# Total-RD/pymgrid

Hardware: AMD Instinct MI355X
Metric: microgrid env-steps/sec (higher is better)
Workload: dtype f64

## Files before the change

### pymgrid_amd/csrc/mgx_core.hpp

```cpp
#pragma once

#include <hip/hip_runtime.h>
#include <stdint.h>

#include "../../include/mgx.h"

namespace mgx {

enum : int { F_GENSET = 1, F_BATTERY = 2, F_GRID = 4, F_GRID_FIRST = 8 };

enum LogCol : int {
    LC_REWARD = 0, LC_FIXED_PROVIDED, LC_FIXED_ABSORBED, LC_CTRL_PROVIDED, LC_CTRL_ABSORBED,
    LC_OVERALL_PROVIDED, LC_OVERALL_ABSORBED,
    LC_LOAD_MET, LC_RENEWABLE_USED, LC_CURTAILMENT, LC_LOSS_LOAD, LC_OVERGENERATION, LC_UNBALANCED_REWARD,
    LC_COMMON_END,
    LC_GENSET_N = 4, LC_BATTERY_N = 5, LC_GRID_N = 4
};

struct KArgs {
    mgx_columns c;
    int32_t N, T, H, final_step;
    int32_t obs_dim, log_dim;
    int32_t n_load, n_pv;
    int32_t n_genset, n_battery, n_grid;
    int32_t obs_f32;
    int32_t act_f32;
    int32_t obs_state_only;
    int32_t done_bits;
    int32_t obs_colpitch;
    int32_t col_load, col_pv, col_gen, col_bat, col_grid;
    int32_t shaper;
    int32_t noise_increase;
    uint64_t noise_seed;
    int32_t *t_dev;
    int32_t g0, g1;
    const int32_t *grid_final;
    int32_t row_mask;
    int32_t *ep_off, *ep_final;
    int32_t ar_mode;
    int32_t ar_fixed_length, ar_lo, ar_hi, ar_max_length;
    uint64_t ar_seed;
    int32_t *ar_start_io, *ar_length_io, *ar_t0_io;
    void *final_obs;
    int32_t pm_pitch;
};

__device__ __forceinline__ uint8_t done_at(const KArgs &a, int64_t i, int32_t t)
{
    const int32_t fin = a.grid_final ? a.grid_final[i] : a.final_step;
    return (uint8_t)(t >= fin - 1);
}

__device__ __forceinline__ int64_t episode_row(const KArgs &a, int32_t t, int32_t off)
{
    const int64_t row = (int64_t)t + off;
    return row < a.T ? (row < 0 ? 0 : row) : (int64_t)a.T - 1;
}
__device__ __forceinline__ int64_t series_row(const KArgs &a, int64_t i, int32_t t)
{
    return a.ep_off ? episode_row(a, t, a.ep_off[i]) : (int64_t)(t & a.row_mask);
}

__device__ __forceinline__ int32_t resolve_t(const KArgs &a, int32_t t)
{
    if (a.t_dev) {
        const int32_t td = a.t_dev[0] + t;
        if (td >= a.T) { a.t_dev[1] = 1; return a.T - 1; }
        return td;
    }
    return t;
}

__device__ __forceinline__ void advance_counter_in_kernel(const KArgs &a, int32_t k)
{
    if (a.t_dev == nullptr) return;
    __syncthreads();
    if (threadIdx.x == 0) {
        const unsigned prev = atomicAdd((unsigned *)&a.t_dev[2], 1u);
        if (prev == gridDim.x - 1) {
            const int32_t t = __hip_atomic_load(&a.t_dev[0], __ATOMIC_RELAXED, __HIP_MEMORY_SCOPE_AGENT);
            __hip_atomic_store(&a.t_dev[2], 0, __ATOMIC_RELAXED, __HIP_MEMORY_SCOPE_AGENT);
            __hip_atomic_store(&a.t_dev[0], t + k, __ATOMIC_RELEASE, __HIP_MEMORY_SCOPE_AGENT);
        }
    }
}

__device__ __forceinline__ int32_t resolve_t_obs(const KArgs &a, int32_t t) { return a.t_dev ? a.t_dev[0] + t : t; }

__device__ __forceinline__ int32_t resolve_k(const KArgs &a, int32_t t0, int32_t K)
{
    if (a.t_dev && t0 + K > a.T) { a.t_dev[1] = 1; return a.T - t0; }
    return K;
}

struct Params {
    double bat_cmin, bat_cmax, bat_C, bat_D, bat_eta, bat_cost;
    double gen_rmin, gen_rmax, gen_cost, gen_co2, gen_cco2;
    uint32_t gen_times;
    double grid_imp, grid_exp, grid_cco2;
    double ll_cost, og_cost;
};

struct State {
    double charge, soc;
    uint32_t status;
};

struct Derived {
    double bat_lo, bat_sp;
    double gen_sp;
    double grid_lo, grid_sp;
};

struct Inputs {
    double a_goal, a_gen, a_bat, a_grid;
    double load, pv;
    double g_pimp, g_pexp, g_co2, g_stat;
};

struct Outputs {
    double reward;
    double fixed_provided, fixed_absorbed, ctrl_provided, ctrl_absorbed, overall_provided, overall_absorbed;
    double load_met, renewable_used, curtailment, loss_load, overgeneration, unbalanced_reward;
    double genset_production, genset_co2, genset_reward;
    double discharge_amount, charge_amount, battery_reward, soc_pre, charge_pre;
    double grid_import, grid_export, grid_co2, grid_reward;
    uint32_t violations;
};

__device__ __forceinline__ double space_spread(double lo, double hi)
{
    double s = hi - lo;
    return s == 0.0 ? 1.0 : s;
}
__device__ __forceinline__ double space_denorm(double lo, double hi, double v) { return lo + space_spread(lo, hi) * v; }
__device__ __forceinline__ double space_norm(double lo, double hi, double v) { return (v - lo) / space_spread(lo, hi); }

__device__ __forceinline__ double py_min(double a, double b)
{
    double r;
    asm("v_min_f64 %0, %1, %2" : "=v"(r) : "v"(a), "v"(b));
    return r;
}
__device__ __forceinline__ double py_max(double a, double b)
{
    double r;
    asm("v_max_f64 %0, %1, %2" : "=v"(r) : "v"(a), "v"(b));
    return r;
}
__device__ __forceinline__ double py_clip(double x, double lo, double hi) { return py_min(py_max(x, lo), hi); }

template <int F>
__device__ __forceinline__ void derive(const Params &p, Derived &d)
{
    if constexpr (F & F_BATTERY) {
        d.bat_lo = -p.bat_D / p.bat_eta;
        d.bat_sp = space_spread(d.bat_lo, p.bat_C * p.bat_eta);
    }
    if constexpr (F & F_GENSET) d.gen_sp = space_spread(0.0, p.gen_rmax);
    if constexpr (F & F_GRID) {
        d.grid_lo = -1 * p.grid_exp;
        d.grid_sp = space_spread(d.grid_lo, p.grid_imp);
    }
}

constexpr int PP = MGX_PROFILE_PITCH;

__host__ __device__ __forceinline__ bool factorised(const mgx_columns &c) { return c.base_load != nullptr; }

struct GridFactors {
    double lr, pr;
    uint32_t lp, pp, cp, pat;
};

template <int F>
__device__ __forceinline__ void load_factors(const mgx_columns &c, int64_t i, GridFactors &f)
{
// ... 117 lines not shown
}

template <int F>
__device__ __forceinline__ void store_state(const mgx_columns &c, int64_t i, const State &s)
{
    if constexpr (F & F_BATTERY) { c.charge[i] = s.charge; c.soc[i] = s.soc; }
    if constexpr (F & F_GENSET) c.gen_status[i] = s.status;
}

template <int F, typename AT>
__device__ __forceinline__ void load_inputs(const mgx_columns &c, const AT *__restrict__ act,
                                            int64_t N, int64_t i, int64_t t, Inputs &in, int32_t pm = 0)
{
    constexpr int A = 2 * ((F & F_GENSET) != 0) + ((F & F_BATTERY) != 0) + ((F & F_GRID) != 0);
    const AT *a = act + i * A;
    int k = 0;
    if constexpr (F & F_GENSET) { in.a_goal = a[k]; in.a_gen = a[k + 1]; k += 2; }
    if constexpr (F & F_BATTERY) { in.a_bat = a[k]; k += 1; }
    if constexpr (F & F_GRID) { in.a_grid = a[k]; k += 1; }
    if (factorised(c)) {
        GridFactors f;
        load_factors<F>(c, i, f);
        fact_series<F>(c, N, i, t, f, in, pm);
        return;
    }
    if (pm) {
        constexpr int C = (F & F_GRID) ? 6 : 2;
        in.load = c.load_ts[ts_index(pm, N, t, i, C)];
        in.pv = c.pv_ts[ts_index(pm, N, t, i, C)];
        in.g_stat = 1.0;
        if constexpr (F & F_GRID) {
            const double *g = c.grid_ts + grid_ts_index(pm, N, t, 0, i);
            in.g_pimp = g[0]; in.g_pexp = g[1]; in.g_co2 = g[2]; in.g_stat = g[3];
        }
        return;
    }
    in.load = c.load_ts[t * N + i];
    in.pv = c.pv_ts[t * N + i];
    in.g_stat = 1.0;
    if constexpr (F & F_GRID) {
        const double *g = c.grid_ts + (t * 4) * N + i;
        in.g_pimp = g[0]; in.g_pexp = g[N]; in.g_co2 = g[2 * N]; in.g_stat = g[3 * N];
    }
}

__device__ __forceinline__ uint32_t genset_update_status(uint32_t st, uint32_t times, double goal_f)
{
    int cur = st & 0xff, gs = (st >> 8) & 0xff, up = (st >> 16) & 0xff, down = st >> 24;
    const int su = times & 0xff, wd = (times >> 16) & 0xff;
    const bool allow = ((times >> 8) & 1u) == 0;
    const int goal = goal_f > 0.5 ? 1 : 0;
    if (!(goal == cur && cur == gs)) {
        const bool instant = (su == 0 && goal == 1) || (wd == 0 && goal == 0);
        if (goal != gs && (allow || instant)) gs = goal;
        bool finished = false;
        if (up == 0 && gs == 1)        { cur = 1; up = 0;   down = wd; finished = true; }
        else if (down == 0 && gs == 0) { cur = 0; down = 0; up = su;   finished = true; }
        if (!finished) {
            if (goal == cur && cur != gs && allow) {
                gs = goal;
                if (cur) { up = 0; down = wd; } else { down = 0; up = su; }
            } else if (cur == gs && gs != goal) {
                if (cur) { up = 0; down = wd; } else { down = 0; up = su; }
                gs = goal;
            }
            if (gs != cur) { if (gs == 0) down -= 1; else up -= 1; }
        }
    }
    return (uint32_t)cur | ((uint32_t)gs << 8) | ((uint32_t)(up & 0xff) << 16) | ((uint32_t)(down & 0xff) << 24);
}

__device__ __forceinline__ int genset_next_status(uint32_t st, int goal)
{
    const int cur = st & 0xff, up = (st >> 16) & 0xff, down = st >> 24;
    if (goal) return (cur || up == 0) ? 1 : 0;
    return (!cur || down == 0) ? 0 : 1;
}

template <int F>
__device__ __forceinline__ bool genset_wave_is_instant(const Params &p, const State &s)
{
    if constexpr (F & F_GENSET)
        return __all((p.gen_times == 0u) && (s.status == 0u || s.status == 0x0101u)) != 0;
    return false;
}

__device__ __forceinline__ double battery_max_production(const Params &p, double charge)
{
    const double b = charge - p.bat_cmin;
    return py_min(p.bat_D, b) * p.bat_eta;
}
__device__ __forceinline__ double battery_max_consumption(const Params &p, double charge)
{
    const double b = p.bat_cmax - charge;
    return py_min(p.bat_C, b) / p.bat_eta;
}

template <int F, bool HAVE_Q = false>
__device__ __forceinline__ void step_core(const Params &p, const Derived &d, State &s, const Inputs &in, bool normalized,
                                          bool want_soc, bool gen_instant, Outputs &o, double bat_q = 0.0)
{
    double prov = 0.0, absb = 0.0, reward = 0.0;
    uint32_t viol = 0u;

    const double L = -1 * in.load;
    o.load_met = L;
    absb += L; reward += 0.0;
    o.fixed_provided = prov; o.fixed_absorbed = absb;

    if constexpr (F & F_GENSET) {
        if (gen_instant) {
            const uint32_t g = in.a_goal > 0.5 ? 1u : 0u;
            s.status = g | (g << 8);
        } else {
            s.status = genset_update_status(s.status, p.gen_times, in.a_goal);
        }
        const double x = normalized ? 0.0 + d.gen_sp * in.a_gen : in.a_gen;
        const double cur = (double)(s.status & 0xff);
        const double mx = cur * p.gen_rmax, mn = cur * p.gen_rmin;
        const double e = py_clip(x, mn, mx);
        viol |= ((x > mx) || (x < mn) ? 1u : 0u) | (!(in.a_goal >= 0.0 && in.a_goal <= 1.0) ? 8u : 0u) | (x < 0.0 ? 16u : 0u);
        const double co2 = p.gen_co2 * e;
        const double cost = p.gen_cost * e + p.gen_cco2 * co2;
        o.genset_production = e; o.genset_co2 = co2; o.genset_reward = -1.0 * cost;
        prov += e; reward += o.genset_reward;
    }

    auto step_battery = [&]() __attribute__((always_inline)) {
        const double x = normalized ? d.bat_lo + d.bat_sp * in.a_bat : in.a_bat;
        o.soc_pre = s.soc; o.charge_pre = s.charge;
        const bool sink = x < 0;
        const double room = p.bat_cmax - s.charge;
        const double num_sink = py_min(p.bat_C, room);
        const double mp = battery_max_production(p, s.charge);
        const double e_src = py_clip(x, 0.0, mp);
        const double num = sink ? num_sink : -1.0 * e_src;
        double q;
        if constexpr (HAVE_Q) q = bat_q; else q = num / p.bat_eta;
        const double ex = -1.0 * x;
        const double e_sink = py_min(ex, q);
        const double e = sink ? e_sink : e_src;
        viol |= (sink ? (ex > q) : (x > mp)) ? 2u : 0u;
        viol |= !((sink ? e_sink : e_src) >= 0) ? 32u : 0u;
        const double internal = sink ? e * p.bat_eta : ((num < 0) ? q : num * p.bat_eta);
        o.charge_amount = sink ? e : 0.0;
        o.discharge_amount = sink ? 0.0 : e;
        absb += o.charge_amount; prov += o.discharge_amount;
        s.charge = py_max(s.charge + internal, p.bat_cmin);
        if (want_soc) s.soc = s.charge / p.bat_cmax;
        o.battery_reward = -1.0 * (fabs(internal) * p.bat_cost);
        reward += o.battery_reward;
    };
    auto step_grid = [&]() __attribute__((always_inline)) {
        const double x = normalized ? d.grid_lo + d.grid_sp * in.a_grid : in.a_grid;
        const bool sink = x < 0;
        const double ex = -1.0 * x, mc = p.grid_exp * in.g_stat;
        const double e_exp = py_min(ex, mc);
        const double mp = p.grid_imp * in.g_stat;
        const double e_imp = py_clip(x, 0.0, mp);
        viol |= (sink ? (ex > mc) : (x > mp)) ? 4u : 0u;
        viol |= !((sink ? e_exp : e_imp) >= 0) ? 32u : 0u;
        const double co2 = sink ? 0.0 : e_imp * in.g_co2;
        const double cco2 = -1.0 * p.grid_cco2 * co2;
        o.grid_export = sink ? e_exp : 0.0;
        o.grid_import = sink ? 0.0 : e_imp;
        o.grid_co2 = co2;
// ... 1203 lines not shown
```

### pymgrid_amd/csrc/mgx_kernels.hpp

```cpp
#pragma once
#include "mgx_core.hpp"

#include <type_traits>

namespace mgx {

#ifndef MGX_BLOCK
#define MGX_BLOCK 128
#endif
constexpr int BLOCK = MGX_BLOCK;
#ifndef MGX_RING
#define MGX_RING 8
#endif
#ifndef MGX_RING_RICH
#define MGX_RING_RICH 16
#endif
#ifndef MGX_BLOCK_K
#define MGX_BLOCK_K 256
#endif
constexpr int BLOCK_K = MGX_BLOCK_K;
#ifndef MGX_RING_ROLLOUT
#define MGX_RING_ROLLOUT 8
#endif

// ... 168 lines not shown
__global__ __launch_bounds__(BLOCK) void step_kernel(const KArgs a, const void *__restrict__ actions, int32_t t,
                                                     int normalized, double *__restrict__ reward,
                                                     uint8_t *__restrict__ done, void *__restrict__ obs,
                                                     double *__restrict__ log)
{
    t = resolve_t(a, t);
    extern __shared__ __attribute__((aligned(16))) double row_tiles[];
    const int64_t i = (int64_t)a.g0 + (int64_t)blockIdx.x * BLOCK + threadIdx.x;
    if (i < a.g1) step_body<F, EP>(a, actions, t, normalized, reward, done, obs, log, i, row_tiles + (threadIdx.x >> 6) * (64 * ROW_TILE_MAX_D));
    advance_counter_in_kernel(a, 1);
}

template <int F>
__global__ __launch_bounds__(BLOCK) void check_kernel(const KArgs a, const void *__restrict__ actions, int32_t t, int normalized,
                                                      uint32_t *__restrict__ violations)
{
    t = resolve_t(a, t);
    const int64_t i = (int64_t)a.g0 + (int64_t)blockIdx.x * BLOCK + threadIdx.x;
    if (i >= a.g1) return;
    Params p; State s; Inputs in; Outputs o; Derived d;
    load_state<F>(a.c, i, true, s);
    load_params<F>(a.c, i, p);
    derive<F>(p, d);
    const int64_t row = series_row(a, i, t);
    if (a.act_f32) load_inputs<F>(a.c, (const float *)actions, a.N, i, row, in, a.pm_pitch);
    else load_inputs<F>(a.c, (const double *)actions, a.N, i, row, in, a.pm_pitch);
    step_core<F>(p, d, s, in, normalized != 0, false, false, o);
    violations[i] = o.violations;
}

struct FusedOut {
    double *reward;
    uint8_t *done;
    double *soc_trace;
    uint32_t *status_trace;
    double *ret_acc;
    double *log;
};

template <typename AT>
struct RawInputs {
    AT a_goal, a_gen, a_bat, a_grid;
    double load, pv, g_pimp, g_pexp, g_co2, g_stat;
};

template <int F, typename AT>
__device__ __forceinline__ Inputs widen(const RawInputs<AT> &r)
{
    Inputs in;
    if constexpr (F & F_GENSET) { in.a_goal = (double)r.a_goal; in.a_gen = (double)r.a_gen; }
    if constexpr (F & F_BATTERY) in.a_bat = (double)r.a_bat;
    if constexpr (F & F_GRID) {
        in.a_grid = (double)r.a_grid;
        in.g_pimp = r.g_pimp; in.g_pexp = r.g_pexp; in.g_co2 = r.g_co2; in.g_stat = r.g_stat;
    }
    in.load = r.load; in.pv = r.pv;
    return in;
}

template <int F, typename AT>
__device__ __forceinline__ void load_inputs_at(const AT *__restrict__ act, const double *__restrict__ lts,
                                               const double *__restrict__ pts, const double *__restrict__ gts,
                                               int64_t N, int64_t i, int64_t off, RawInputs<AT> &in)
{
    constexpr int A = 2 * ((F & F_GENSET) != 0) + ((F & F_BATTERY) != 0) + ((F & F_GRID) != 0);
    const AT *a = act + off * A;
    int k = 0;
    if constexpr (F & F_GENSET) { in.a_goal = a[k]; in.a_gen = a[k + 1]; k += 2; }
    if constexpr (F & F_BATTERY) { in.a_bat = a[k]; k += 1; }
    if constexpr (F & F_GRID) { in.a_grid = a[k]; k += 1; }
    in.load = lts[off];
    in.pv = pts[off];
    if constexpr (F & F_GRID) {
        const double *g = gts + (4 * off - 3 * i);
        in.g_pimp = g[0]; in.g_pexp = g[N]; in.g_co2 = g[2 * N]; in.g_stat = g[3 * N];
    }
}

#ifndef MGX_FACT_ROWS
#define MGX_FACT_ROWS 128
#endif
constexpr int FACT_ROWS = MGX_FACT_ROWS;

template <int F>
__device__ __forceinline__ void stage_base_rows(const mgx_columns &c, int64_t row0, int32_t n, double *lds, int nthreads)
{
    const int32_t cnt = n * PP;
    const double *__restrict__ bl = c.base_load + row0 * PP;
    const double *__restrict__ bp = c.base_pv + row0 * PP;
    for (int32_t j = threadIdx.x; j < cnt; j += nthreads) {
        lds[j] = bl[j];
        lds[FACT_ROWS * PP + j] = bp[j];
        if constexpr (F & F_GRID) lds[2 * FACT_ROWS * PP + j] = c.base_co2[row0 * PP + j];
    }
}

struct BaseVals { double load, pv, co2; };

template <int F>
__device__ __forceinline__ BaseVals read_base_row(const double *lds, int32_t r, const GridFactors &f)
{
    BaseVals b;
    b.load = lds[r * PP + f.lp];
    b.pv = lds[FACT_ROWS * PP + r * PP + f.pp];
    b.co2 = 0.0;
    if constexpr (F & F_GRID) b.co2 = lds[2 * FACT_ROWS * PP + r * PP + f.cp];
    return b;
}

struct OutageWords {
    uint64_t cur, nxt;
    int64_t wi;
};

__device__ __forceinline__ void outage_init(const mgx_columns &c, int64_t N, int64_t i, int32_t T, int32_t t0, OutageWords &w)
{
    w.wi = t0 >> 6; w.cur = 0; w.nxt = 0;
    if (c.outage_bits) {
        w.cur = c.outage_bits[w.wi * N + i];
        if ((w.wi + 1) * 64 < T) w.nxt = c.outage_bits[(w.wi + 1) * N + i];
    }
}

__device__ __forceinline__ double outage_status(const mgx_columns &c, int64_t N, int64_t i, int32_t T, int32_t row, bool first,
                                                OutageWords &w)
{
    if (!first && (row & 63) == 0) {
        w.cur = w.nxt; w.wi += 1; w.nxt = 0;
        if (c.outage_bits && (w.wi + 1) * 64 < T) w.nxt = c.outage_bits[(w.wi + 1) * N + i];
    }
    return ((w.cur >> (row & 63)) & 1ull) ? 0.0 : 1.0;
}

template <typename AT>
struct RawActions {
    AT a_goal, a_gen, a_bat, a_grid;
};

template <int F, typename AT>
__device__ __forceinline__ void load_actions_at(const AT *__restrict__ row, uint32_t i32, RawActions<AT> &r)
{
    constexpr int A = 2 * ((F & F_GENSET) != 0) + ((F & F_BATTERY) != 0) + ((F & F_GRID) != 0);
    const AT *a = row + i32 * (uint32_t)A;
    int k = 0;
#if MGX_ACT_NT
    if constexpr (F & F_GENSET) { r.a_goal = __builtin_nontemporal_load(a + k); r.a_gen = __builtin_nontemporal_load(a + k + 1); k += 2; }
    if constexpr (F & F_BATTERY) { r.a_bat = __builtin_nontemporal_load(a + k); k += 1; }
    if constexpr (F & F_GRID) { r.a_grid = __builtin_nontemporal_load(a + k); k += 1; }
#else
    if constexpr (F & F_GENSET) { r.a_goal = a[k]; r.a_gen = a[k + 1]; k += 2; }
    if constexpr (F & F_BATTERY) { r.a_bat = a[k]; k += 1; }
    if constexpr (F & F_GRID) { r.a_grid = a[k]; k += 1; }
#endif
}

__device__ __forceinline__ void store_done(const KArgs &a, uint8_t *__restrict__ done, int64_t off, int64_t i, int32_t k, bool dn)
{
    if (a.done_bits) {
        const unsigned long long b = __ballot(dn);
        const int lane = threadIdx.x & 63;
        if ((lane & 15) == 0) {
            const int64_t W = ((int64_t)a.N + 15) >> 4;
            reinterpret_cast<uint16_t *>(done)[(int64_t)k * W + (i >> 4)] = (uint16_t)(b >> (lane & 48));
        }
    } else {
        done[off] = (uint8_t)dn;
    }
}

template <int F, int U, typename AT, bool RICH, bool FACT>
__global__ __launch_bounds__(BLOCK_K) void step_k_kernel(const KArgs a, const AT *__restrict__ actions, int32_t t0,
                                                         int32_t K, int normalized, const FusedOut out_rt, int32_t gpb)
{
    FusedOut out = out_rt;
    if constexpr (!RICH) { out.log = nullptr; out.status_trace = nullptr; }
    const int32_t K_launch = K;
    t0 = resolve_t(a, t0);
    K = resolve_k(a, t0, K);
    const int64_t i = (int64_t)a.g0 + (int64_t)blockIdx.x * gpb + threadIdx.x;
    const bool active = (int32_t)threadIdx.x < gpb && i < a.g1;
    if constexpr (!FACT) { if (!active) return; }
    const int64_t N = a.N;
    constexpr int A_DIM = 2 * ((F & F_GENSET) != 0) + ((F & F_BATTERY) != 0) + ((F & F_GRID) != 0);
    Params p; State s; Derived d;
    const bool norm = normalized != 0;
    const bool want_soc = (out.soc_trace != nullptr) || (out.log != nullptr);
    bool gen_instant = false;
    int32_t k_done = 0;
    if (active) {
        load_state<F>(a.c, i, out.log != nullptr, s);
        load_params<F>(a.c, i, p);
        derive<F>(p, d);
        gen_instant = genset_wave_is_instant<F>(p, s);
        k_done = (a.grid_final ? a.grid_final[i] : a.final_step) - 1 - t0;
    }
    double ret = 0.0;

    const bool hot = !RICH && out.reward != nullptr && out.done == nullptr && (!(F & F_BATTERY) || out.soc_trace != nullptr) &&
                     a.shaper == MGX_SHAPER_NONE;
    const uint32_t i32 = (uint32_t)i;
    auto consume = [&](auto gi_tag, auto hot_tag, const Inputs &in, int32_t k, int64_t off) __attribute__((always_inline)) {
        constexpr bool GI = decltype(gi_tag)::value, HOT = decltype(hot_tag)::value;
        Outputs o;
        step_core<F>(p, d, s, in, norm, HOT ? (F & F_BATTERY) != 0 : want_soc, GI, o);
        if constexpr (HOT) {
            const double r = o.reward;
#if MGX_HOT_NT
            __builtin_nontemporal_store(r, (out.reward + (int64_t)k * N) + i32);
            if constexpr (F & F_BATTERY) __builtin_nontemporal_store(s.soc, (out.soc_trace + (int64_t)k * N) + i32);
#else
            (out.reward + (int64_t)k * N)[i32] = r;
            if constexpr (F & F_BATTERY) (out.soc_trace + (int64_t)k * N)[i32] = s.soc;
#endif
            ret += r;
            return;
        }
        const double r = shaped_reward<F>(a.shaper, o);
        {
#if MGX_OUT_NT
            if (out.reward) __builtin_nontemporal_store(r, out.reward + off);
            if (out.done) store_done(a, out.done, off, i, k, k >= k_done);
            if constexpr (F & F_BATTERY) { if (out.soc_trace) __builtin_nontemporal_store(s.soc, out.soc_trace + off); }
            if constexpr (F & F_GENSET) { if (out.status_trace) __builtin_nontemporal_store(s.status, out.status_trace + off); }
#else
            if (out.reward) out.reward[off] = r;
            if (out.done) store_done(a, out.done, off, i, k, k >= k_done);
            if constexpr (F & F_BATTERY) { if (out.soc_trace) out.soc_trace[off] = s.soc; }
            if constexpr (F & F_GENSET) { if (out.status_trace) out.status_trace[off] = s.status; }
#endif
            if (out.log) store_log<F>(out.log + (off - i) * a.log_dim + i, N, o, s.status);
        }
        ret += r;
    };
    auto specialised = [&](auto fn) __attribute__((always_inline)) {
        if constexpr ((F & F_GENSET) != 0) {
            if (gen_instant) { if (hot) fn(std::true_type{}, std::true_type{}); else fn(std::true_type{}, std::false_type{}); }
            else { if (hot) fn(std::false_type{}, std::true_type{}); else fn(std::false_type{}, std::false_type{}); }
        } else {
            if (hot) fn(std::false_type{}, std::true_type{}); else fn(std::false_type{}, std::false_type{});
        }
    };

    if constexpr (FACT) {
        __shared__ double base_lds[((F & F_GRID) ? 3 : 2) * FACT_ROWS * PP];
        static_assert(FACT_ROWS % U == 0, "ring slots are addressed by k % U across LDS chunks");
        GridFactors f;
        f.lr = 0.0; f.pr = 0.0; f.lp = 0u; f.pp = 0u; f.cp = 0u; f.pat = 0u;
        OutageWords ow;
        ow.cur = 0; ow.nxt = 0; ow.wi = 0;
        RawActions<AT> ring[U];
        if (active) {
            load_factors<F>(a.c, i, f);
            if constexpr (F & F_GRID) outage_init(a.c, N, i, a.T, t0, ow);
#pragma unroll
            for (int u = 0; u < U; u++)
                if (u < K) load_actions_at<F>(actions + (int64_t)u * N * A_DIM, i32, ring[u]);
        }
        int64_t off = i;
        auto run_chunk = [&](auto gi_tag, auto hot_tag, int32_t kb, int32_t n) __attribute__((always_inline)) {
            BaseVals nb = read_base_row<F>(base_lds, 0, f);
            for (int32_t k0 = kb; k0 < kb + n; k0 += U) {
#pragma unroll
                for (int u = 0; u < U; u++) {
                    const int32_t k = k0 + u;
                    if (k < kb + n) {
                        const RawActions<AT> ra = ring[u];
                        if (k + U < K) load_actions_at<F>(actions + (int64_t)(k + U) * N * A_DIM, i32, ring[u]);
                        Inputs in;
                        if constexpr (F & F_GENSET) { in.a_goal = (double)ra.a_goal; in.a_gen = (double)ra.a_gen; }
                        if constexpr (F & F_BATTERY) in.a_bat = (double)ra.a_bat;
                        in.load = fact_load(nb.load, f.lr);
                        in.pv = fact_pv(nb.pv, f.pr);
                        if constexpr (F & F_GRID) {
                            in.a_grid = (double)ra.a_grid;
                            in.g_pimp = tariff_price((int32_t)f.pat, t0 + k); in.g_pexp = 0.0;
                            in.g_co2 = nb.co2;
                            in.g_stat = outage_status(a.c, N, i, a.T, t0 + k, k == 0, ow);
                        }
                        const int32_t rn = (k + 1 - kb < n) ? k + 1 - kb : n - 1;
                        nb = read_base_row<F>(base_lds, rn, f);
                        consume(gi_tag, hot_tag, in, k, off);
                        off += N;
                    }
                }
            }
        };
        for (int32_t kb = 0; kb < K; kb += FACT_ROWS) {
            const int32_t n = K - kb < FACT_ROWS ? K - kb : FACT_ROWS;
            __syncthreads();
            stage_base_rows<F>(a.c, (int64_t)t0 + kb, n, base_lds, BLOCK_K);
            __syncthreads();
            if (active) specialised([&](auto gi_tag, auto hot_tag) __attribute__((always_inline)) { run_chunk(gi_tag, hot_tag, kb, n); });
        }
        if (!active) return;
    } else {
        const double *__restrict__ lts = a.c.load_ts + (int64_t)t0 * N;
        const double *__restrict__ pts = a.c.pv_ts + (int64_t)t0 * N;
        const double *__restrict__ gts = (F & F_GRID) ? a.c.grid_ts + (int64_t)t0 * 4 * N : nullptr;
        specialised([&](auto gi_tag, auto hot_tag) __attribute__((always_inline)) {
            RawInputs<AT> ring[U];
#pragma unroll
            for (int u = 0; u < U; u++)
                if (u < K) load_inputs_at<F>(actions, lts, pts, gts, N, i, (int64_t)u * N + i, ring[u]);

            int64_t off = i;
            for (int32_t k0 = 0; k0 < K; k0 += U) {
#pragma unroll
                for (int u = 0; u < U; u++) {
                    const int32_t k = k0 + u;
                    if (k < K) {
                        const Inputs in = widen<F>(ring[u]);
                        if (k + U < K) load_inputs_at<F>(actions, lts, pts, gts, N, i, off + (int64_t)U * N, ring[u]);
                        consume(gi_tag, hot_tag, in, k, off);
                        off += N;
                    }
                }
            }
        });
    }
    if constexpr (F & F_BATTERY) { if (!want_soc) s.soc = s.charge / p.bat_cmax; }
    store_state<F>(a.c, i, s);
    if (out.ret_acc) out.ret_acc[i] += ret;
    advance_counter_in_kernel(a, K_launch);
}

struct FusedLaunch {
    int flags;
    bool act_f32, rich, fact, per_step;
    unsigned blocks;
    hipStream_t stream;
    const KArgs *k;
    const void *actions;
    const PLWords *tab;
    const uint8_t *ids;
    int32_t t, K;
    int normalized;
    FusedOut out;
    int32_t gpb;
};
constexpr int MGX_FUSED_PARTS = 6;
struct MultiStaticLaunch {
    int flags, ng, nb, nr, nl, np;
    unsigned blocks;
    hipStream_t stream;
    const KArgs *k;
    const void *actions;
    int32_t t, K;
    int normalized;
    FusedOut out;
};
bool launch_step_k_multi_static(const MultiStaticLaunch &L);
struct MultiStaticRollout {
    int flags, ng, nb, nr, nl, np;
    unsigned blocks;
    hipStream_t stream;
    const KArgs *k;
    const int32_t *lists;
    int32_t n_lists, list_len;
    const int32_t *ids;
    int per_step;
    int32_t t, K;
    FusedOut out;
};
bool launch_rollout_multi_static(const MultiStaticRollout &L);
bool launch_step_k_p0(const FusedLaunch &L); bool launch_step_k_p1(const FusedLaunch &L); bool launch_step_k_p2(const FusedLaunch &L);
bool launch_step_k_p3(const FusedLaunch &L); bool launch_step_k_p4(const FusedLaunch &L);
bool launch_rollout_p0(const FusedLaunch &L); bool launch_rollout_p1(const FusedLaunch &L); bool launch_rollout_p2(const FusedLaunch &L);
bool launch_rollout_p3(const FusedLaunch &L); bool launch_rollout_p4(const FusedLaunch &L);
enum : int { EP_SRC_FACT = 0, EP_SRC_GRID_MAJOR = 1, EP_SRC_GATHER = 2 };
struct EpisodeLaunch {
    int flags;
    int src;
    bool per_step;
    unsigned blocks;
    int32_t gpb;
    hipStream_t stream;
    const KArgs *k;
    const KArgs *k_dev;
    const PLWords *tab;
    const uint8_t *ids;
    int32_t t, K;
    FusedOut out;
    mgx_episode_stats stats;
};
constexpr int MGX_EPISODE_PARTS = 2;
bool launch_rollout_episodes_p0(const EpisodeLaunch &L); bool launch_rollout_episodes_p1(const EpisodeLaunch &L);
struct StepEpisodeLaunch {
    int flags;
    int src;
    bool act_f32;
    unsigned blocks;
    int32_t gpb;
    hipStream_t stream;
    const KArgs *k;
    const KArgs *k_dev;
    const void *actions;
    int32_t t, K;
    int normalized;
    FusedOut out;
    mgx_episode_stats stats;
};
constexpr int MGX_STEP_EPISODE_PARTS = 2;
bool launch_step_k_episodes_p0(const StepEpisodeLaunch &L); bool launch_step_k_episodes_p1(const StepEpisodeLaunch &L);

template <int F>
// ... 707 lines not shown
#define MGX_FLEET_CASE(FV) case FV: step_discrete_body<FV>(a, tab, (const int32_t *)actions, t, nullptr, reward, done, obs, log, i); break;
        switch (flags) {
            MGX_FLEET_CASE(0) MGX_FLEET_CASE(1) MGX_FLEET_CASE(2) MGX_FLEET_CASE(3) MGX_FLEET_CASE(4)
            MGX_FLEET_CASE(5) MGX_FLEET_CASE(6) MGX_FLEET_CASE(7) MGX_FLEET_CASE(14)
            default: step_discrete_body<15>(a, tab, (const int32_t *)actions, t, nullptr, reward, done, obs, log, i); break;
        }
#undef MGX_FLEET_CASE
        return;
    }
#define MGX_FLEET_CASE(FV) case FV: step_body<FV>(a, actions, t, fa.normalized, reward, done, obs, log, i); break;
    switch (flags) {
        MGX_FLEET_CASE(0) MGX_FLEET_CASE(1) MGX_FLEET_CASE(2) MGX_FLEET_CASE(3) MGX_FLEET_CASE(4)
        MGX_FLEET_CASE(5) MGX_FLEET_CASE(6) MGX_FLEET_CASE(7) MGX_FLEET_CASE(14)
        default: step_body<15>(a, actions, t, fa.normalized, reward, done, obs, log, i); break;
    }
#undef MGX_FLEET_CASE
}

struct FleetHead {
    const PLWords *tab;
    int64_t n_grids;
    int32_t t, flags, pad0, pad1;
};
struct FleetBucket {
    FleetHead hd;
    KArgs k;
    const void *actions;
    double *reward; uint8_t *done; void *obs; double *log;
};
struct FleetArgsV {
    int32_t n, normalized, pad0, pad1;
    FleetBucket b[MGX_FLEET_MAX];
};
static_assert(sizeof(FleetArgsV) <= 3840, "the kernarg segment holds 4 KB");

#define MGX_FLEET_V_HEAD \
    typedef const char __attribute__((address_space(4))) *kernarg_bytes; \
    const kernarg_bytes mine = (kernarg_bytes)__builtin_amdgcn_kernarg_segment_ptr() + offsetof(FleetArgsV, b) \
                               + (size_t)blockIdx.y * sizeof(FleetBucket); \
    typedef uint32_t u32x8 __attribute__((ext_vector_type(8))); \
    static_assert(sizeof(FleetHead) == 32 && offsetof(FleetBucket, hd) == 0, "the head is one s_load_dwordx8"); \
    const u32x8 h8 = *reinterpret_cast<const u32x8 __attribute__((address_space(4))) *>(mine); \
    FleetHead hd; \
    hd.tab = reinterpret_cast<const PLWords *>((uint64_t)h8[0] | ((uint64_t)h8[1] << 32)); \
    hd.n_grids = (int64_t)((uint64_t)h8[2] | ((uint64_t)h8[3] << 32)); \
    hd.t = (int32_t)h8[4]; hd.flags = (int32_t)h8[5]; \
    const int64_t i = (int64_t)blockIdx.x * BLOCK + threadIdx.x; \
    if (i >= hd.n_grids) return; \
    const int normalized = fa.normalized; \
    const FleetBucket &B = *reinterpret_cast<const FleetBucket *>((const char *)mine);

#define MGX_FLEET_V_DISCRETE(FV, EPV) case FV: { step_discrete_body<FV, EPV>(B.k, *hd.tab, (const int32_t *)B.actions, hd.t, nullptr, B.reward, B.done, B.obs, B.log, i); } break;
#define MGX_FLEET_V_STEP(FV, EPV) case FV: { step_body<FV, EPV>(B.k, B.actions, hd.t, normalized, B.reward, B.done, B.obs, B.log, i); } break;
#define MGX_FLEET_V_SWITCHES(EPV)                                                                                                     \
    if (hd.tab != nullptr) {                                  \
        switch (hd.flags) {                                                                                                           \
            MGX_FLEET_V_DISCRETE(0, EPV) MGX_FLEET_V_DISCRETE(1, EPV) MGX_FLEET_V_DISCRETE(2, EPV) MGX_FLEET_V_DISCRETE(3, EPV)       \
            MGX_FLEET_V_DISCRETE(4, EPV) MGX_FLEET_V_DISCRETE(5, EPV) MGX_FLEET_V_DISCRETE(6, EPV) MGX_FLEET_V_DISCRETE(7, EPV)       \
            MGX_FLEET_V_DISCRETE(14, EPV)                                                                                             \
            default: { step_discrete_body<15, EPV>(B.k, *hd.tab, (const int32_t *)B.actions, hd.t, nullptr, B.reward, B.done, B.obs, B.log, i); } break; \
        }                                                                                                                             \
        return;                                                                                                                       \
    }                                                                                                                                 \
    switch (hd.flags) {                                                                                                               \
        MGX_FLEET_V_STEP(0, EPV) MGX_FLEET_V_STEP(1, EPV) MGX_FLEET_V_STEP(2, EPV) MGX_FLEET_V_STEP(3, EPV) MGX_FLEET_V_STEP(4, EPV)   \
        MGX_FLEET_V_STEP(5, EPV) MGX_FLEET_V_STEP(6, EPV) MGX_FLEET_V_STEP(7, EPV) MGX_FLEET_V_STEP(14, EPV)                          \
        default: { step_body<15, EPV>(B.k, B.actions, hd.t, normalized, B.reward, B.done, B.obs, B.log, i); } break;                  \
    }

template <bool EP>
static __global__ __launch_bounds__(BLOCK) void fleet_step_kernel_v(const FleetArgsV fa)
{
    MGX_FLEET_V_HEAD
    MGX_FLEET_V_SWITCHES(EP)
}

template <int F, int U, bool PER_STEP, bool RICH, bool FACT>
__global__ __launch_bounds__(BLOCK_K) void rollout_kernel(const KArgs a, const PLWords tab, const uint8_t *__restrict__ ids,
                                                          int32_t t0, int32_t K, const FusedOut out_rt, int32_t gpb)
{
    FusedOut out = out_rt;
    if constexpr (!RICH) { out.log = nullptr; out.status_trace = nullptr; }
    const int32_t K_launch = K;
    t0 = resolve_t(a, t0);
    K = resolve_k(a, t0, K);
    const int64_t i = (int64_t)a.g0 + (int64_t)blockIdx.x * gpb + threadIdx.x;
    const bool active = (int32_t)threadIdx.x < gpb && i < a.g1;
    if constexpr (!FACT) { if (!active) return; }
    const int64_t N = a.N;
    Params p; State s; Derived d;
    const bool want_soc = (out.soc_trace != nullptr) || (out.log != nullptr);
    bool gen_instant = false;
    int32_t k_done = 0;
    uint32_t word = 0u;
    if (active) {
        load_state<F>(a.c, i, out.log != nullptr, s);
        load_params<F>(a.c, i, p);
        derive<F>(p, d);
        gen_instant = genset_wave_is_instant<F>(p, s);
        k_done = (a.grid_final ? a.grid_final[i] : a.final_step) - 1 - t0;
        word = PER_STEP ? 0u : pl_select(tab, ids[i]);
    }
    double ret = 0.0;

    const bool hot = !RICH && out.reward != nullptr && out.done == nullptr && (!(F & F_BATTERY) || out.soc_trace != nullptr) &&
                     a.shaper == MGX_SHAPER_NONE;
    const uint32_t i32 = (uint32_t)i;
    auto consume = [&](auto gi_tag, auto hot_tag, Inputs &in, int32_t k, int64_t off) __attribute__((always_inline)) {
        constexpr bool GI = decltype(gi_tag)::value, HOT = decltype(hot_tag)::value;
        double bat_q;
        uint32_t xv = 0u;
        populate_core<F, RICH>(p, s, word, in, bat_q, 0.0 + -1 * in.load, in.pv, GI, &xv);
        Outputs o;
        step_core<F, true>(p, d, s, in, false, HOT ? (F & F_BATTERY) != 0 : want_soc, GI, o, bat_q);
        if constexpr (RICH) o.violations |= xv;
        if constexpr (HOT) {
            const double r = o.reward;
            (out.reward + (int64_t)k * N)[i32] = r;
            if constexpr (F & F_BATTERY) (out.soc_trace + (int64_t)k * N)[i32] = s.soc;
            ret += r;
            return;
        }
        const double r = shaped_reward<F>(a.shaper, o);
        if (out.reward) out.reward[off] = r;
        if (out.done) store_done(a, out.done, off, i, k, k >= k_done);
        if constexpr (F & F_BATTERY) { if (out.soc_trace) out.soc_trace[off] = s.soc; }
        if constexpr (F & F_GENSET) { if (out.status_trace) out.status_trace[off] = s.status; }
        if (out.log) store_log<F>(out.log + (off - i) * a.log_dim + i, N, o, s.status);
        ret += r;
    };
    auto specialised = [&](auto fn) __attribute__((always_inline)) {
        if constexpr ((F & F_GENSET) != 0) {
            if (gen_instant) { if (hot) fn(std::true_type{}, std::true_type{}); else fn(std::true_type{}, std::false_type{}); }
            else { if (hot) fn(std::false_type{}, std::true_type{}); else fn(std::false_type{}, std::false_type{}); }
        } else {
            if (hot) fn(std::false_type{}, std::true_type{}); else fn(std::false_type{}, std::false_type{});
        }
    };
    if constexpr (FACT) {
        __shared__ double base_lds[((F & F_GRID) ? 3 : 2) * FACT_ROWS * PP];
        static_assert(FACT_ROWS % U == 0, "ring slots are addressed by k % U across LDS chunks");
        GridFactors f;
        f.lr = 0.0; f.pr = 0.0; f.lp = 0u; f.pp = 0u; f.cp = 0u; f.pat = 0u;
        OutageWords ow;
        ow.cur = 0; ow.nxt = 0; ow.wi = 0;
        static_assert(U <= 8, "the id ring is one 64-bit register");
        uint64_t idq = 0;
        if (active) {
            load_factors<F>(a.c, i, f);
            if constexpr (F & F_GRID) outage_init(a.c, N, i, a.T, t0, ow);
            if constexpr (PER_STEP) {
#pragma unroll
                for (int u = 0; u < U; u++)
                    if (u < K) idq |= (uint64_t)(ids + (int64_t)u * N)[i32] << (8 * u);
            }
        }
        int64_t off = i;
        auto run_chunk = [&](auto gi_tag, auto hot_tag, int32_t kb, int32_t n) __attribute__((always_inline)) {
            BaseVals nb = read_base_row<F>(base_lds, 0, f);
            for (int32_t k0 = kb; k0 < kb + n; k0 += U) {
#pragma unroll
                for (int u = 0; u < U; u++) {
                    const int32_t k = k0 + u;
                    if (k < kb + n) {
                        if constexpr (PER_STEP) {
                            word = pl_select(tab, (int32_t)((idq >> (8 * u)) & 0xffu));
                            if (k + U < K)
                                idq = (idq & ~(0xffull << (8 * u))) | ((uint64_t)(ids + (int64_t)(k + U) * N)[i32] << (8 * u));
                        }
                        Inputs in;
                        in.load = fact_load(nb.load, f.lr);
                        in.pv = fact_pv(nb.pv, f.pr);
                        in.g_stat = 1.0;
                        if constexpr (F & F_GRID) {
                            in.g_pimp = tariff_price((int32_t)f.pat, t0 + k); in.g_pexp = 0.0;
                            in.g_co2 = nb.co2;
                            in.g_stat = outage_status(a.c, N, i, a.T, t0 + k, k == 0, ow);
                        }
                        const int32_t rn = (k + 1 - kb < n) ? k + 1 - kb : n - 1;
                        nb = read_base_row<F>(base_lds, rn, f);
                        consume(gi_tag, hot_tag, in, k, off);
                        off += N;
                    }
                }
            }
        };
        for (int32_t kb = 0; kb < K; kb += FACT_ROWS) {
            const int32_t n = K - kb < FACT_ROWS ? K - kb : FACT_ROWS;
            __syncthreads();
            stage_base_rows<F>(a.c, (int64_t)t0 + kb, n, base_lds, BLOCK_K);
            __syncthreads();
            if (active) specialised([&](auto gi_tag, auto hot_tag) __attribute__((always_inline)) { run_chunk(gi_tag, hot_tag, kb, n); });
        }
        if (!active) return;
    } else {
        specialised([&](auto gi_tag, auto hot_tag) __attribute__((always_inline)) {
            const double *__restrict__ lts = a.c.load_ts + (int64_t)t0 * N;
            const double *__restrict__ pts = a.c.pv_ts + (int64_t)t0 * N;
            const double *__restrict__ gts = (F & F_GRID) ? a.c.grid_ts + (int64_t)t0 * 4 * N : nullptr;
            Inputs ring[U];
            uint8_t idr[U];
#pragma unroll
            for (int u = 0; u < U; u++)
                if (u < K) {
                    load_series_at<F>(lts, pts, gts, N, i, (int64_t)u * N + i, ring[u]);
                    if constexpr (PER_STEP) idr[u] = ids[(int64_t)u * N + i];
                }

            int64_t off = i;
            for (int32_t k0 = 0; k0 < K; k0 += U) {
#pragma unroll
                for (int u = 0; u < U; u++) {
                    const int32_t k = k0 + u;
                    if (k < K) {
                        Inputs in = ring[u];
                        if constexpr (PER_STEP) word = pl_select(tab, idr[u]);
                        if (k + U < K) {
                            load_series_at<F>(lts, pts, gts, N, i, off + (int64_t)U * N, ring[u]);
                            if constexpr (PER_STEP) idr[u] = ids[off + (int64_t)U * N];
                        }
                        consume(gi_tag, hot_tag, in, k, off);
                        off += N;
                    }
                }
            }
        });
    }
    if constexpr (F & F_BATTERY) { if (!want_soc) s.soc = s.charge / p.bat_cmax; }
    store_state<F>(a.c, i, s);
    if (out.ret_acc) out.ret_acc[i] += ret;
    advance_counter_in_kernel(a, K_launch);
}

constexpr int BLOCK_MULTI = 64;

__device__ __forceinline__ StepLists multi_lists(const KArgs &a, double *lds)
{
    const int cap = multi_list_capacity(a.n_load, a.n_pv, a.n_genset, a.n_battery, a.n_grid);
    StepLists L;
    L.stride = BLOCK_MULTI; L.n_prov = 0; L.n_absb = 0;
    L.prov = lds + threadIdx.x;
    L.absb = lds + (size_t)cap * BLOCK_MULTI + threadIdx.x;
    return L;
}

template <typename OT>
__device__ __forceinline__ void observe_series_multi(const double *__restrict__ ts, int64_t row_stride, int32_t T, int32_t t, int32_t H,
                                                     double lo, double hi, OT *__restrict__ obs, int obs_stride = 1, bool noisy = false,
                                                     double noise_std = 0.0, uint64_t noise_seed = 0, int noise_increase = 0,
                                                     int64_t grid = 0, uint32_t comp = 0)
{
    const double fill = (hi + lo) / 2, sp = space_spread(lo, hi);
    for (int h = 0; h <= H; h++) {
        const bool in = t < T && t + h < T;
        double v = in ? ts[(int64_t)(t + h) * row_stride] : 0.0;
        if (noisy && in && h > 0) {
            const double sd = noise_increase ? noise_std * (1.0 + log(1.0 + (double)(h - 1))) : noise_std;
            v += sd * forecast_normal(noise_seed, grid, comp, t, h);
        }
        obs[h * obs_stride] = (OT)obs_series_value(v, in, h > 0, lo, hi, fill, sp);
    }
}

template <int F, typename OT>
__device__ inline void observe_state_multi(const KArgs &a, int64_t i, OT *__restrict__ dst, int64_t stride)
{
    const int64_t N = a.N;
    int64_t k = 0;
    if constexpr (F & F_GENSET) {
        for (int j = 0; j < a.n_genset; j++) {
            const int64_t c = (int64_t)j * N + i;
            const uint32_t times = a.c.gen_times[c], st = a.c.gen_status[c];
            const double su = (double)(times & 0xff), wd = (double)((times >> 16) & 0xff);
            dst[(k++) * stride] = (OT)space_norm(0.0, 1.0, (double)(st & 0xff));
            dst[(k++) * stride] = (OT)space_norm(0.0, 1.0, (double)((st >> 8) & 0xff));
            dst[(k++) * stride] = (OT)space_norm(0.0, su, (double)((st >> 16) & 0xff));
            dst[(k++) * stride] = (OT)space_norm(0.0, wd, (double)(st >> 24));
        }
    }
    if constexpr (F & F_BATTERY) {
        for (int j = 0; j < a.n_battery; j++) {
            const int64_t c = (int64_t)j * N + i;
            const double cmin = a.c.bat_min_capacity[c], cmax = a.c.bat_max_capacity[c];
            dst[(k++) * stride] = (OT)space_norm(cmin / cmax, 1.0, a.c.soc[c]);
            dst[(k++) * stride] = (OT)space_norm(cmin, cmax, a.c.charge[c]);
        }
    }
}

template <int F, typename OT, bool NOISE = false>
__device__ inline void observe_row_multi(const KArgs &a, int64_t i, int32_t t, OT *__restrict__ obs_row)
{
    const int64_t N = a.N;
    const int W = 1 + a.H;
    int k = (a.n_load + a.n_pv) * W;
    observe_state_multi<F, OT>(a, i, obs_row + k, 1);
    if (a.obs_state_only) return;
    k = 0;
    const uint64_t nseed = a.noise_seed;
    const int ninc = a.noise_increase;
    for (int j = 0; j < a.n_load; j++, k += W) {
        const bool noisy = NOISE && a.c.load_noise_std != nullptr;
        const double sd = noisy ? a.c.load_noise_std[(int64_t)j * N + i] : 0.0;
        observe_series_multi(a.c.load_ts + (int64_t)j * N + i, (int64_t)a.n_load * N, a.T, t, a.H, a.c.load_lo[(int64_t)j * N + i],
                             a.c.load_hi[(int64_t)j * N + i], obs_row + k, 1, noisy, sd, nseed, ninc, i, (uint32_t)j);
    }
    for (int j = 0; j < a.n_pv; j++, k += W) {
        const bool noisy = NOISE && a.c.pv_noise_std != nullptr;
        const double sd = noisy ? a.c.pv_noise_std[(int64_t)j * N + i] : 0.0;
        observe_series_multi(a.c.pv_ts + (int64_t)j * N + i, (int64_t)a.n_pv * N, a.T, t, a.H, a.c.pv_lo[(int64_t)j * N + i],
                             a.c.pv_hi[(int64_t)j * N + i], obs_row + k, 1, noisy, sd, nseed, ninc, i, (uint32_t)(MGX_MAX_MODULES + j));
    }
    k += 4 * a.n_genset + 2 * a.n_battery;
// ... 1010 lines not shown
```

Baseline: 134.7 billion.

## Hoist prologue loads and base-row staging ahead of state init

Issues the first LDS chunk's global loads into registers at kernel entry. State, params, factors, outage words, action/id rings and ret_acc are then all loaded unconditionally, with inactive lanes clamped to the last valid index, so every load goes out before the first use. This is meant to overlap prologue memory latency and drop the leading barrier. The range and overrun resolution becomes branchless and the overrun flag is written at the end. In exchange it uses more registers for the staged rows, and inactive lanes do redundant loads.

```diff
diff --git a/pymgrid_amd/csrc/mgx_core.hpp b/pymgrid_amd/csrc/mgx_core.hpp
--- a/pymgrid_amd/csrc/mgx_core.hpp
+++ b/pymgrid_amd/csrc/mgx_core.hpp
@@ -93,6 +93,29 @@
     return K;
 }
 
+struct LaunchRange {
+    int32_t t0, K;
+    bool overrun;
+};
+__device__ __forceinline__ LaunchRange resolve_range(const KArgs &a, int32_t t, int32_t K)
+{
+    const bool dc = a.t_dev != nullptr;
+    int32_t tv = 0;
+    if (dc) tv = a.t_dev[0];
+    const int32_t td = tv + t;
+    const bool over_t = dc && td >= a.T;
+    LaunchRange r;
+    r.t0 = over_t ? a.T - 1 : td;
+    const bool over_k = dc && r.t0 + K > a.T;
+    r.K = over_k ? a.T - r.t0 : K;
+    r.overrun = over_t || over_k;
+    return r;
+}
+__device__ __forceinline__ void flag_overrun(const KArgs &a, const LaunchRange &r)
+{
+    if (r.overrun) a.t_dev[1] = 1;
+}
+
 struct Params {
     double bat_cmin, bat_cmax, bat_C, bat_D, bat_eta, bat_cost;
     double gen_rmin, gen_rmax, gen_cost, gen_co2, gen_cco2;
@@ -376,6 +399,13 @@
 {
     if constexpr (F & F_GENSET)
         return __all((p.gen_times == 0u) && (s.status == 0u || s.status == 0x0101u)) != 0;
+    return false;
+}
+template <int F>
+__device__ __forceinline__ bool genset_wave_is_instant(const Params &p, const State &s, bool active)
+{
+    if constexpr (F & F_GENSET)
+        return __all(!active || ((p.gen_times == 0u) && (s.status == 0u || s.status == 0x0101u))) != 0;
     return false;
 }
 
diff --git a/pymgrid_amd/csrc/mgx_kernels.hpp b/pymgrid_amd/csrc/mgx_kernels.hpp
--- a/pymgrid_amd/csrc/mgx_kernels.hpp
+++ b/pymgrid_amd/csrc/mgx_kernels.hpp
@@ -274,16 +274,40 @@
 #endif
 constexpr int FACT_ROWS = MGX_FACT_ROWS;
 
+constexpr int STAGE_PER_THREAD = FACT_ROWS * PP / BLOCK_K;
+static_assert(FACT_ROWS * PP % BLOCK_K == 0, "every thread stages the same number of elements of a chunk");
+
 template <int F>
-__device__ __forceinline__ void stage_base_rows(const mgx_columns &c, int64_t row0, int32_t n, double *lds, int nthreads)
-{
-    const int32_t cnt = n * PP;
+struct StagedRows {
+    double load[STAGE_PER_THREAD], pv[STAGE_PER_THREAD], co2[(F & F_GRID) ? STAGE_PER_THREAD : 1];
+};
+
+template <int F>
+__device__ __forceinline__ void stage_load(const mgx_columns &c, int64_t row0, int32_t n, StagedRows<F> &r)
+{
+    const int32_t last = n * PP - 1;
     const double *__restrict__ bl = c.base_load + row0 * PP;
     const double *__restrict__ bp = c.base_pv + row0 * PP;
-    for (int32_t j = threadIdx.x; j < cnt; j += nthreads) {
-        lds[j] = bl[j];
-        lds[FACT_ROWS * PP + j] = bp[j];
-        if constexpr (F & F_GRID) lds[2 * FACT_ROWS * PP + j] = c.base_co2[row0 * PP + j];
+    const double *__restrict__ bc = (F & F_GRID) ? c.base_co2 + row0 * PP : nullptr;
+#pragma unroll
+    for (int m = 0; m < STAGE_PER_THREAD; m++) {
+        const int32_t j = (int32_t)threadIdx.x + m * BLOCK_K;
+        const int32_t jj = j < last ? j : last;
+        r.load[m] = bl[jj];
+        r.pv[m] = bp[jj];
+        if constexpr (F & F_GRID) r.co2[m] = bc[jj];
+    }
+}
+
+template <int F>
+__device__ __forceinline__ void stage_store(const StagedRows<F> &r, double *lds)
+{
+#pragma unroll
+    for (int m = 0; m < STAGE_PER_THREAD; m++) {
+        const int32_t j = (int32_t)threadIdx.x + m * BLOCK_K;
+        lds[j] = r.load[m];
+        lds[FACT_ROWS * PP + j] = r.pv[m];
+        if constexpr (F & F_GRID) lds[2 * FACT_ROWS * PP + j] = r.co2[m];
     }
 }
 
@@ -367,25 +391,45 @@
     FusedOut out = out_rt;
     if constexpr (!RICH) { out.log = nullptr; out.status_trace = nullptr; }
     const int32_t K_launch = K;
-    t0 = resolve_t(a, t0);
-    K = resolve_k(a, t0, K);
+    const LaunchRange lr = resolve_range(a, t0, K);
+    t0 = lr.t0; K = lr.K;
     const int64_t i = (int64_t)a.g0 + (int64_t)blockIdx.x * gpb + threadIdx.x;
     const bool active = (int32_t)threadIdx.x < gpb && i < a.g1;
     if constexpr (!FACT) { if (!active) return; }
+    const int64_t il = (FACT && i >= a.g1) ? (int64_t)a.g1 - 1 : i;
+    const uint32_t il32 = (uint32_t)il;
     const int64_t N = a.N;
     constexpr int A_DIM = 2 * ((F & F_GENSET) != 0) + ((F & F_BATTERY) != 0) + ((F & F_GRID) != 0);
     Params p; State s; Derived d;
     const bool norm = normalized != 0;
     const bool want_soc = (out.soc_trace != nullptr) || (out.log != nullptr);
-    bool gen_instant = false;
-    int32_t k_done = 0;
-    if (active) {
-        load_state<F>(a.c, i, out.log != nullptr, s);
-        load_params<F>(a.c, i, p);
-        derive<F>(p, d);
-        gen_instant = genset_wave_is_instant<F>(p, s);
-        k_done = (a.grid_final ? a.grid_final[i] : a.final_step) - 1 - t0;
-    }
+    StagedRows<F> staged;
+    if constexpr (FACT) stage_load<F>(a.c, t0, K < FACT_ROWS ? K : FACT_ROWS, staged);
+    load_state<F>(a.c, il, false, s);
+    if constexpr (RICH && (F & F_BATTERY)) {
+        const double soc0 = a.c.soc[il];
+        s.soc = out.log ? soc0 : 0.0;
+    }
+    load_params<F>(a.c, il, p);
+    int32_t fin = a.final_step;
+    if (a.grid_final) fin = a.grid_final[il];
+    double ret0 = 0.0;
+    if constexpr (FACT) { if (out.ret_acc) ret0 = out.ret_acc[il]; }
+    GridFactors f;
+    f.lr = 0.0; f.pr = 0.0; f.lp = 0u; f.pp = 0u; f.cp = 0u; f.pat = 0u;
+    OutageWords ow;
+    ow.cur = 0; ow.nxt = 0; ow.wi = 0;
+    RawActions<AT> ring[FACT ? U : 1];
+    if constexpr (FACT) {
+        load_factors<F>(a.c, il, f);
+        if constexpr (F & F_GRID) outage_init(a.c, N, il, a.T, t0, ow);
+#pragma unroll
+        for (int u = 0; u < U; u++)
+            if (u < K) load_actions_at<F>(actions + (int64_t)u * N * A_DIM, il32, ring[u]);
+    }
+    derive<F>(p, d);
+    const bool gen_instant = genset_wave_is_instant<F>(p, s, active);
+    const int32_t k_done = fin - 1 - t0;
     double ret = 0.0;
 
     const bool hot = !RICH && out.reward != nullptr && out.done == nullptr && (!(F & F_BATTERY) || out.soc_trace != nullptr) &&
@@ -436,18 +480,8 @@
     if constexpr (FACT) {
         __shared__ double base_lds[((F & F_GRID) ? 3 : 2) * FACT_ROWS * PP];
         static_assert(FACT_ROWS % U == 0, "ring slots are addressed by k % U across LDS chunks");
-        GridFactors f;
-        f.lr = 0.0; f.pr = 0.0; f.lp = 0u; f.pp = 0u; f.cp = 0u; f.pat = 0u;
-        OutageWords ow;
-        ow.cur = 0; ow.nxt = 0; ow.wi = 0;
-        RawActions<AT> ring[U];
-        if (active) {
-            load_factors<F>(a.c, i, f);
-            if constexpr (F & F_GRID) outage_init(a.c, N, i, a.T, t0, ow);
-#pragma unroll
-            for (int u = 0; u < U; u++)
-                if (u < K) load_actions_at<F>(actions + (int64_t)u * N * A_DIM, i32, ring[u]);
-        }
+        stage_store<F>(staged, base_lds);
+        __syncthreads();
         int64_t off = i;
         auto run_chunk = [&](auto gi_tag, auto hot_tag, int32_t kb, int32_t n) __attribute__((always_inline)) {
             BaseVals nb = read_base_row<F>(base_lds, 0, f);
@@ -479,9 +513,12 @@
         };
         for (int32_t kb = 0; kb < K; kb += FACT_ROWS) {
             const int32_t n = K - kb < FACT_ROWS ? K - kb : FACT_ROWS;
-            __syncthreads();
-            stage_base_rows<F>(a.c, (int64_t)t0 + kb, n, base_lds, BLOCK_K);
-            __syncthreads();
+            if (kb > 0) {
+                stage_load<F>(a.c, (int64_t)t0 + kb, n, staged);
+                __syncthreads();
+                stage_store<F>(staged, base_lds);
+                __syncthreads();
+            }
             if (active) specialised([&](auto gi_tag, auto hot_tag) __attribute__((always_inline)) { run_chunk(gi_tag, hot_tag, kb, n); });
         }
         if (!active) return;
@@ -512,7 +549,11 @@
     }
     if constexpr (F & F_BATTERY) { if (!want_soc) s.soc = s.charge / p.bat_cmax; }
     store_state<F>(a.c, i, s);
-    if (out.ret_acc) out.ret_acc[i] += ret;
+    if (out.ret_acc) {
+        if constexpr (!FACT) ret0 = out.ret_acc[i];
+        out.ret_acc[i] = ret0 + ret;
+    }
+    flag_overrun(a, lr);
     advance_counter_in_kernel(a, K_launch);
 }
 
@@ -1386,25 +1427,49 @@
     FusedOut out = out_rt;
     if constexpr (!RICH) { out.log = nullptr; out.status_trace = nullptr; }
     const int32_t K_launch = K;
-    t0 = resolve_t(a, t0);
-    K = resolve_k(a, t0, K);
+    const LaunchRange lr = resolve_range(a, t0, K);
+    t0 = lr.t0; K = lr.K;
     const int64_t i = (int64_t)a.g0 + (int64_t)blockIdx.x * gpb + threadIdx.x;
     const bool active = (int32_t)threadIdx.x < gpb && i < a.g1;
     if constexpr (!FACT) { if (!active) return; }
+    const int64_t il = (FACT && i >= a.g1) ? (int64_t)a.g1 - 1 : i;
+    const uint32_t il32 = (uint32_t)il;
     const int64_t N = a.N;
     Params p; State s; Derived d;
     const bool want_soc = (out.soc_trace != nullptr) || (out.log != nullptr);
-    bool gen_instant = false;
-    int32_t k_done = 0;
-    uint32_t word = 0u;
-    if (active) {
-        load_state<F>(a.c, i, out.log != nullptr, s);
-        load_params<F>(a.c, i, p);
-        derive<F>(p, d);
-        gen_instant = genset_wave_is_instant<F>(p, s);
-        k_done = (a.grid_final ? a.grid_final[i] : a.final_step) - 1 - t0;
-        word = PER_STEP ? 0u : pl_select(tab, ids[i]);
-    }
+    StagedRows<F> staged;
+    if constexpr (FACT) stage_load<F>(a.c, t0, K < FACT_ROWS ? K : FACT_ROWS, staged);
+    load_state<F>(a.c, il, false, s);
+    if constexpr (RICH && (F & F_BATTERY)) {
+        const double soc0 = a.c.soc[il];
+        s.soc = out.log ? soc0 : 0.0;
+    }
+    load_params<F>(a.c, il, p);
+    int32_t fin = a.final_step;
+    if (a.grid_final) fin = a.grid_final[il];
+    double ret0 = 0.0;
+    if constexpr (FACT) { if (out.ret_acc) ret0 = out.ret_acc[il]; }
+    uint8_t id_fixed = 0;
+    if constexpr (!PER_STEP) id_fixed = ids[il];
+    GridFactors f;
+    f.lr = 0.0; f.pr = 0.0; f.lp = 0u; f.pp = 0u; f.cp = 0u; f.pat = 0u;
+    OutageWords ow;
+    ow.cur = 0; ow.nxt = 0; ow.wi = 0;
+    static_assert(!FACT || U <= 8, "the id ring is one 64-bit register");
+    uint64_t idq = 0;
+    if constexpr (FACT) {
+        load_factors<F>(a.c, il, f);
+        if constexpr (F & F_GRID) outage_init(a.c, N, il, a.T, t0, ow);
+        if constexpr (PER_STEP) {
+#pragma unroll
+            for (int u = 0; u < U; u++)
+                if (u < K) idq |= (uint64_t)(ids + (int64_t)u * N)[il32] << (8 * u);
+        }
+    }
+    derive<F>(p, d);
+    const bool gen_instant = genset_wave_is_instant<F>(p, s, active);
+    const int32_t k_done = fin - 1 - t0;
+    uint32_t word = PER_STEP ? 0u : pl_select(tab, id_fixed);
     double ret = 0.0;
 
     const bool hot = !RICH && out.reward != nullptr && out.done == nullptr && (!(F & F_BATTERY) || out.soc_trace != nullptr) &&
@@ -1444,21 +1509,8 @@
     if constexpr (FACT) {
         __shared__ double base_lds[((F & F_GRID) ? 3 : 2) * FACT_ROWS * PP];
         static_assert(FACT_ROWS % U == 0, "ring slots are addressed by k % U across LDS chunks");
-        GridFactors f;
-        f.lr = 0.0; f.pr = 0.0; f.lp = 0u; f.pp = 0u; f.cp = 0u; f.pat = 0u;
-        OutageWords ow;
-        ow.cur = 0; ow.nxt = 0; ow.wi = 0;
-        static_assert(U <= 8, "the id ring is one 64-bit register");
-        uint64_t idq = 0;
-        if (active) {
-            load_factors<F>(a.c, i, f);
-            if constexpr (F & F_GRID) outage_init(a.c, N, i, a.T, t0, ow);
-            if constexpr (PER_STEP) {
-#pragma unroll
-                for (int u = 0; u < U; u++)
-                    if (u < K) idq |= (uint64_t)(ids + (int64_t)u * N)[i32] << (8 * u);
-            }
-        }
+        stage_store<F>(staged, base_lds);
+        __syncthreads();
         int64_t off = i;
         auto run_chunk = [&](auto gi_tag, auto hot_tag, int32_t kb, int32_t n) __attribute__((always_inline)) {
             BaseVals nb = read_base_row<F>(base_lds, 0, f);
@@ -1491,9 +1543,12 @@
         };
         for (int32_t kb = 0; kb < K; kb += FACT_ROWS) {
             const int32_t n = K - kb < FACT_ROWS ? K - kb : FACT_ROWS;
-            __syncthreads();
-            stage_base_rows<F>(a.c, (int64_t)t0 + kb, n, base_lds, BLOCK_K);
-            __syncthreads();
+            if (kb > 0) {
+                stage_load<F>(a.c, (int64_t)t0 + kb, n, staged);
+                __syncthreads();
+                stage_store<F>(staged, base_lds);
+                __syncthreads();
+            }
             if (active) specialised([&](auto gi_tag, auto hot_tag) __attribute__((always_inline)) { run_chunk(gi_tag, hot_tag, kb, n); });
         }
         if (!active) return;
@@ -1532,7 +1587,11 @@
     }
     if constexpr (F & F_BATTERY) { if (!want_soc) s.soc = s.charge / p.bat_cmax; }
     store_state<F>(a.c, i, s);
-    if (out.ret_acc) out.ret_acc[i] += ret;
+    if (out.ret_acc) {
+        if constexpr (!FACT) ret0 = out.ret_acc[i];
+        out.ret_acc[i] = ret0 + ret;
+    }
+    flag_overrun(a, lr);
     advance_counter_in_kernel(a, K_launch);
 }
 
```

After: 133.7 billion. No clear change (-0.7%).
